# collabora/WhisperLive

Measured on AMD Instinct MI355X. Metric: real-time factor (xRT), Whisper-small 30 s window (p50 chunk latency in p50_chunk_latency_ms), higher is better.
Workload: dtype f16 (MFMA operands; f32 accumulate, f32 residual stream, f32 log-mel); 1 GPU; configs[1]: Whisper-small.en, 1 stream per GPU, one 30 s window per stream per step (480000 samples 16 kHz f32 resident in HBM -> log-mel -> encoder -> beam-5 decode, 64 generated tokens forced by suppressing EOT), seeded random weights; streams_per_gpu=1, beam_size=5, decode_steps=64

## Files before the change

### whisperlive_amd/_lib.py

```python
from __future__ import annotations

import ctypes as C
import os
import shutil
import subprocess
from pathlib import Path

import numpy as np

PKG_DIR = Path(__file__).resolve().parent
CSRC = PKG_DIR / "csrc"
DEFAULT_LIB = PKG_DIR / "libwlx.so"
LIB_PATH = Path(os.environ["WLX_LIB"]).resolve() if os.environ.get("WLX_LIB") else DEFAULT_LIB
SOURCES = ["pack.hip", "logmel.hip", "gemm.hip", "attention.hip", "decoder.hip", "align.hip", "dec_gemv.hip", "dec_vocab.hip", "search.hip", "host.hip", "engine.hip", "engine_decode.hip", "engine_debug.hip", "resample.hip", "flac.hip", "vad.hip", "mt.hip", "mt_engine.hip", "spk.hip", "spk_engine.hip",
           "kernel_hooks.hip"]
EXPORTS = [
    "wlx_abi_version", "wlx_last_error", "wlx_engine_create", "wlx_engine_destroy", "wlx_engine_spec",
    "wlx_slot_create", "wlx_slot_destroy", "wlx_logmel", "wlx_pcm_put", "wlx_pcm_put_frames", "wlx_pcm_put_frames_split", "wlx_flac_probe", "wlx_pcm_put_flac", "wlx_pcm_put_flac_split", "wlx_pcm_get", "wlx_logmel_resident", "wlx_features_get", "wlx_features_set", "wlx_encode",
    "wlx_encoder_output_get", "wlx_generate", "wlx_generate_ex", "wlx_detect_language", "wlx_align", "wlx_align_batch", "wlx_timings_get", "wlx_sync",
    "wlx_vad_create", "wlx_vad_destroy", "wlx_vad_probs",
    "wlx_ring_create", "wlx_ring_destroy", "wlx_ring_append", "wlx_ring_state", "wlx_vad_probs_resident", "wlx_vad_segments", "wlx_logmel_ring",
    "wlx_logmel_chunks", "wlx_logmel_chunks_multi", "wlx_vad_probs_pcm", "wlx_vad_probs_batch", "wlx_vad_probs_pcm_batch",
    "wlx_mt_create", "wlx_mt_destroy", "wlx_mt_slot_create", "wlx_mt_slot_destroy", "wlx_mt_translate",
    "wlx_spk_create", "wlx_spk_destroy", "wlx_spk_embed", "wlx_spk_embed_batch", "wlx_spk_embed_pcm_batch", "wlx_spk_embed_ring_batch",
    "wlx_debug_logits_get", "wlx_debug_decode_logits", "wlx_debug_search", "wlx_debug_search_batch", "wlx_debug_time_decode_step", "wlx_debug_profile_step", "wlx_debug_trace_step",
    "wlx_mt_debug_encode", "wlx_mt_debug_decode_logits", "wlx_mt_debug_timings", "wlx_mt_debug_attn", "wlx_mt_debug_topk",
    "wlx_mt_debug_embed",
    "wlx_spk_debug_timings", "wlx_spk_debug_fbank", "wlx_spk_debug_conv", "wlx_spk_debug_pool",
    "wlx_spk_debug_conv_batch", "wlx_spk_debug_pool_batch",
    "wlx_debug_layernorm", "wlx_debug_attn_encoder", "wlx_debug_dec_cross_attn", "wlx_debug_dec_self_attn", "wlx_debug_gemm",
    "wlx_debug_dec_gemv", "wlx_debug_dec_cq_cross_attn",
    "wlx_debug_resample", "wlx_debug_resample_split", "wlx_debug_resample_timed", "wlx_debug_flac_decode", "wlx_debug_flac_timings",
    "wlx_debug_dtw", "wlx_debug_align_post", "wlx_debug_align_timings",
]


HIPCC_EXTRA = ["-mllvm", "-amdgpu-mfma-vgpr-form=1"]


class WlxError(RuntimeError):
    code = None


class wlx_spec(C.Structure):
    _fields_ = [(n, C.c_int32) for n in
                ("n_mels", "d_model", "n_heads", "enc_layers", "dec_layers", "ffn", "vocab", "n_audio_ctx", "n_text_ctx")]


class wlx_tensor(C.Structure):
    _fields_ = [("name", C.c_char_p), ("data", C.c_void_p), ("ndim", C.c_int32), ("shape", C.c_int64 * 4),
                ("on_device", C.c_int32)]


class wlx_token_ids(C.Structure):
    _fields_ = [(n, C.c_int32) for n in ("sot", "eot", "no_timestamps", "timestamp_begin", "no_speech", "blank")]


class wlx_gen_opts(C.Structure):
    _fields_ = [
        ("beam_size", C.c_int32), ("patience", C.c_float), ("num_hypotheses", C.c_int32),
        ("length_penalty", C.c_float), ("repetition_penalty", C.c_float), ("no_repeat_ngram_size", C.c_int32),
        ("max_length", C.c_int32), ("suppress_blank", C.c_int32), ("suppress_tokens", C.POINTER(C.c_int32)),
        ("n_suppress_tokens", C.c_int32), ("max_initial_timestamp_index", C.c_int32), ("sampling_topk", C.c_int32),
        ("sampling_temperature", C.c_float), ("seed", C.c_uint64), ("ids", wlx_token_ids),
    ]


class wlx_timings(C.Structure):
    _fields_ = [("logmel_ms", C.c_float), ("encode_ms", C.c_float), ("generate_ms", C.c_float), ("decode_steps", C.c_int32)]

# ... 32 lines not shown
ALIGN_MAX_MEDIAN = 15
ERR_ARG = 1
ERR_STATE = 4
LM_MAXRANGES = 256
PCM_F32, PCM_S16 = 0, 1
PCM_MAX_CHANNELS = 8
RESAMPLE_MAX_RATIO = 640
RESAMPLE_MIN_TILE = 64
RESAMPLE_MAX_LDS = 64 * 1024


class wlx_debug_gemm_args(C.Structure):
    _fields_ = ([(n, C.c_int32) for n in ("zbatch", "M", "N", "K", "KT", "conv3_cin", "mode", "force_form", "d", "rows_per_item")] +
                [("qscale", C.c_float), ("reserved", C.c_int32)] +
                [(n, C.c_int64) for n in ("lda", "strideA", "a_len", "ldc", "strideC", "c_len", "ldx", "strideX", "x_len",
                                          "ldk", "kv_item_stride_k", "kv_layer_stride_k", "k_len",
                                          "ldvt", "kv_item_stride_v", "kv_layer_stride_v", "v_len")])


class wlx_debug_dec_gemv_args(C.Structure):
    _fields_ = ([(n, C.c_int32) for n in ("in_mode", "out_mode", "xsrc", "M", "K", "KT", "N", "busy_device", "KTS", "H", "R", "d")] +
                [("qscale", C.c_float), ("reserved", C.c_int32)] +
                [(n, C.c_int64) for n in ("ldx", "ldxh", "ldyh", "ldy", "ldxres", "cache_row_stride", "slab_stride",
                                          "x_len", "xh_len", "part_o_len", "part_ml_len", "slab_len", "tok_emb_len", "pos_emb_len",
                                          "yh_len", "y_len", "xres_len", "kc_len", "vc_len", "intok_len")])


class wlx_mt_gen_opts(C.Structure):
    _fields_ = [("num_beams", C.c_int32), ("max_length", C.c_int32), ("early_stopping", C.c_int32),
                ("length_penalty", C.c_float), ("no_repeat_ngram_size", C.c_int32), ("forced_eos_token_id", C.c_int32)]


_extra_ok = None


def _hipcc() -> str:
    hipcc = shutil.which("hipcc") or "/opt/rocm/bin/hipcc"
    if not os.path.exists(hipcc):
        raise WlxError("hipcc not found: cannot build libwlx.so (ROCm toolchain required)")
    return hipcc


def _compile(out: Path, defines=(), verbose: bool = False, force: bool = False) -> Path:
    global _extra_ok
    from concurrent.futures import ThreadPoolExecutor
    hipcc = _hipcc()
    defines = list(defines)
    hdrs = list(CSRC.glob("*.h")) + [PKG_DIR.parent / "include" / "wlx.h"]
    hdr_time = max(h.stat().st_mtime for h in hdrs)
    base = [hipcc, "--offload-arch=gfx950", "-O3", "-std=c++17", "-fPIC"] + [f"-D{d}" for d in defines]

    def objects(extra):
        tag = "_".join(["base" if extra else "agpr"] + [d.replace("=", "-") for d in defines])
        odir = CSRC / ".obj" / tag
        odir.mkdir(parents=True, exist_ok=True)

        def one(src):
            obj = odir / (src + ".o")
            sp = CSRC / src
            if not force and obj.exists() and obj.stat().st_mtime >= max(sp.stat().st_mtime, hdr_time):
                return obj, None
            tmp = obj.with_name(obj.name + f".tmp{os.getpid()}")
            proc = subprocess.run(base + extra + ["-c", str(sp), "-o", str(tmp)], capture_output=True, text=True)
            if verbose and (proc.stdout or proc.stderr):
                print(proc.stdout, proc.stderr)
            if proc.returncode != 0:
                if tmp.exists():
                    tmp.unlink()
                return None, proc
            os.replace(tmp, obj)
            return obj, None
        with ThreadPoolExecutor(max_workers=min(len(SOURCES), os.cpu_count() or 4)) as ex:
            return list(ex.map(one, SOURCES))

    for extra in ([HIPCC_EXTRA, []] if _extra_ok is not False else [[]]):
        res = objects(extra)
        bad = [p for o, p in res if o is None]
        if not bad:
            if extra:
                _extra_ok = True
            tmp = out.with_name(out.name + f".tmp{os.getpid()}")
            proc = subprocess.run([hipcc, "--offload-arch=gfx950", "-shared", "-fPIC", "-o", str(tmp)] + [str(o) for o, _ in res],
                                  capture_output=True, text=True)
            if proc.returncode != 0:
                if tmp.exists():
                    tmp.unlink()
                raise WlxError(f"hipcc link failed ({proc.returncode}):\n{proc.stderr[-4000:]}")
            os.replace(tmp, out)
            return out
        err = bad[0].stderr
        if extra and ("Unknown command line argument" in err or "unknown argument" in err.lower()):
            _extra_ok = False
            print(f"[wlx build] this hipcc rejects {' '.join(HIPCC_EXTRA)}: building with MFMA accumulators in AGPR form")
            continue
        raise WlxError(f"hipcc failed ({bad[0].returncode}):\n{err[-4000:]}")
    raise WlxError("hipcc failed")


def _fresh(out: Path) -> bool:
    deps = [CSRC / s for s in SOURCES] + list(CSRC.glob("*.h")) + [PKG_DIR.parent / "include" / "wlx.h"]
    return out.exists() and all(out.stat().st_mtime >= d.stat().st_mtime for d in deps)


def build_trace() -> Path:
    out = PKG_DIR / "libwlx_trace.so"
    return out if _fresh(out) else _compile(out, ["WLX_TRACE"])


def build_ab() -> Path:
    out = PKG_DIR / "libwlx_ab.so"
    return out if _fresh(out) else _compile(out, ["WLX_AB"])


def build_variant(name: str, defines) -> Path:
    out = PKG_DIR / name
    return out if _fresh(out) else _compile(out, list(defines))


def build(force: bool = False, verbose: bool = False) -> Path:
    if not force and _fresh(DEFAULT_LIB):
        return DEFAULT_LIB
    return _compile(DEFAULT_LIB, (), verbose, force=force)


_lib = None


def load() -> C.CDLL:
    global _lib
    if _lib is not None:
        return _lib
    if not LIB_PATH.exists():
        raise WlxError(f"{LIB_PATH} not built: run `python -c 'import __graft_entry__ as g; g.build()'` "
                       "(hipcc --offload-arch=gfx950). whisperlive_amd has no CPU fallback.")
    try:
        lib = C.CDLL(str(LIB_PATH))
    except OSError as e:
        raise WlxError(f"cannot load {LIB_PATH}: {e}") from e
    missing = [s for s in EXPORTS if not hasattr(lib, s)]
    if missing:
        raise WlxError(f"libwlx.so lacks symbols {missing}")
    i32, i64, f32p, i32p, vp = C.c_int32, C.c_int64, C.POINTER(C.c_float), C.POINTER(C.c_int32), C.c_void_p
    lib.wlx_abi_version.restype = i32
    lib.wlx_last_error.restype = C.c_char_p
    lib.wlx_engine_create.argtypes = [C.POINTER(wlx_spec), C.POINTER(wlx_tensor), i32, i32, C.POINTER(vp)]
    lib.wlx_engine_destroy.argtypes = [vp]
    lib.wlx_engine_destroy.restype = None
    lib.wlx_engine_spec.argtypes = [vp, C.POINTER(wlx_spec)]
    lib.wlx_slot_create.argtypes = [vp, i32, i32, i32p]
# ... 131 lines not shown
```

### whisperlive_amd/csrc/dec_gemv.hip

```cpp
#include "dec_gemv_internal.h"
#include <algorithm>
#include <cstdio>

namespace wlx {

#define GV_CH 6

template <int MT, int NTB, int IN>
__global__ __launch_bounds__(512) void dec_gemv_kernel(GemvParams p) {
    if (p.done && *p.done) return;
    extern __shared__ __attribute__((aligned(16))) float smem[];
    const int tid = threadIdx.x, wave = tid >> 6, lane = tid & 63, c = lane & 15, g = lane >> 4;
    const int nw = blockDim.x >> 6;
    const int KT = p.KT;
    const int KTW = (KT + nw - 1) / nw;
    const int kt0 = wave * KTW;
    const int kt1 = (kt0 + KTW < KT) ? kt0 + KTW : KT;
    const int NT_total = (p.N + 15) >> 4;

    const half_t* wbase[NTB];
#pragma unroll
    for (int i = 0; i < NTB; ++i) {
        int nt = blockIdx.x * NTB + i;
        if (nt >= NT_total) nt = NT_total - 1;
// ... 290 lines not shown
template <int P, class F>
__device__ __forceinline__ void stage_rows_f16_wave(const half_t* __restrict__ X, long ldx, int M, int K, half_t* xs, int ldxs, int lane,
                                                    F&& after_first_loads) {
    const int kv8 = K >> 3, total = M * kv8;
    {
        int m_[P], k_[P];
        f16x8 v_[P];
#pragma unroll
        for (int q = 0; q < P; ++q) {
            int u = lane + 64 * q;
            if (u >= total) u = (q == 0) ? total - 1 : (lane + 64 * (q - 1) < total ? lane + 64 * (q - 1) : total - 1);
            m_[q] = u / kv8; k_[q] = u - m_[q] * kv8;
            v_[q] = ld_f16x8(X + (long)m_[q] * ldx + k_[q] * 8);
        }
        after_first_loads();
#pragma unroll
        for (int q = 0; q < P; ++q) *reinterpret_cast<f16x8*>(xs + m_[q] * ldxs + k_[q] * 8) = v_[q];
    }
#pragma unroll 1
    for (int u0 = lane + 64 * P; u0 < total; u0 += 128) {
        const int u1 = u0 + 64;
        const int m0 = u0 / kv8, k0 = u0 - m0 * kv8;
        const int uc = (u1 < total) ? u1 : u0;
        const int m1 = uc / kv8, k1 = uc - m1 * kv8;
        const f16x8 v0 = ld_f16x8(X + (long)m0 * ldx + k0 * 8);
        const f16x8 v1 = ld_f16x8(X + (long)m1 * ldx + k1 * 8);
        *reinterpret_cast<f16x8*>(xs + m0 * ldxs + k0 * 8) = v0;
        *reinterpret_cast<f16x8*>(xs + m1 * ldxs + k1 * 8) = v1;
    }
}


template <int CH, int LNV, int IN, int OUT, int NTB, int MT, int XS>
__global__ __launch_bounds__((IN == GEMV_IN_LN || OUT == GEMV_OUT_SLAB || MT > 1 || CH > 6 || IN == GEMV_IN_XATTN) ? 512 : 1024) void dec_gemv2_kernel(GemvParams p_in) {
    GemvParams p = p_in;
    int tile = blockIdx.x;
    if (p_in.Mtot > 0) {
        int zc = (int)blockIdx.z;
        if (p_in.rt_nz > 0) {
            const int lin = (int)blockIdx.x, t = lin >> 3;
            const int tq = (int)(((unsigned)t * (unsigned)p_in.rt_magic) >> 16);
            zc = t - tq * p_in.rt_nz;
            tile = tq * 8 + (lin & 7);
            if (tile >= p_in.rt_tiles) return;
        }
        const int CHK = p_in.chunk;
        const int r0 = zc * CHK;
        p.M = (p_in.Mtot - r0 < CHK) ? p_in.Mtot - r0 : CHK;
        if (p.emb_token) p.emb_token += r0;
        if (p.X) p.X += (long)r0 * p.ldx;
        if (p.Xh) p.Xh += (long)r0 * p.ldxh;
        if (p.Yh) p.Yh += (long)r0 * p.ldyh;
        if (p.Y) p.Y += (long)r0 * p.ldy;
        if (p.Xres) p.Xres += (long)r0 * p.ldxres;
        if (p.slab) p.slab += (long)r0 * ((IN == GEMV_IN_LN) ? p.ldx : p.ldxres);
        if (p.row_cache) p.row_cache += r0;
        if (p.row_pos) p.row_pos += r0;
    }
    static_assert(XS == GEMV_X_PLAIN || IN == GEMV_IN_LN || (IN == GEMV_IN_F16 && OUT == GEMV_OUT_RESID && NTB == 1),
                  "slab / embedding sources: LayerNorm prologue or residual epilogue only");
    static_assert(OUT != GEMV_OUT_SLAB || (IN == GEMV_IN_F16 && NTB == 1), "K-split form: fp16 rows in");
    extern __shared__ __attribute__((aligned(16))) float smem[];
    const int tid = threadIdx.x, lane = tid & 63, c = lane & 15, g = lane >> 4;
    const int wave = __builtin_amdgcn_readfirstlane(tid >> 6);
    const int nw = p.nwm;
    WLX_TR_BEGIN();
    constexpr int NP = NTB * MT;
    constexpr bool LNT = (LNV == 15);
    constexpr int NV = LNT ? 2 : LNV;
    const bool tail_on = !LNT || lane < 32;
    const int tback = LNT ? (tail_on ? 0 : lane) : 0;
    (void)tail_on; (void)tback;
    float* accred = smem;
    half_t* xs = reinterpret_cast<half_t*>(smem + nw * NP * 256);

    const bool streams = (IN != GEMV_IN_XATTN) || wave < nw;
    const int kx0 = (streams ? wave : 0) * p.KTW;
    const int ks0 = (OUT == GEMV_OUT_SLAB) ? (int)blockIdx.y * p.KTS : 0;
    const int kw0 = ks0 + kx0;
    const half_t* wp = p.Wp + ((long)(tile * NTB) * p.KT + kw0) * 512 + lane * 8;
    const long wstep = (long)p.KT * 512;
    f16x8 wf[CH][NTB];
    auto load_weights = [&]() {
        asm volatile("" ::: "memory");
        const half_t* wq = streams ? wp : p.Wp + ((long)(tile * NTB) * p.KT + ks0) * 512 + lane * 8;
        const long js = streams ? 512 : 0, is = streams ? wstep : 0;
#pragma unroll
        for (int j = 0; j < CH; ++j)
#pragma unroll
            for (int i = 0; i < NTB; ++i) wf[j][i] = ld_nt_f16x8(wq + i * is + j * js);
    };

    int crow[MT];
#pragma unroll
    for (int mt = 0; mt < MT; ++mt) crow[mt] = (mt * 16 + c < p.M) ? mt * 16 + c : p.M - 1;
    const int pair0 = (wave < NP) ? wave : 0;
    const int nt_e = tile * NTB + pair0 / MT;
    const int n_e = nt_e * 16 + g * 4;
    int row_e = (pair0 % MT) * 16 + c;
    if (row_e >= p.M) row_e = p.M - 1;
    float4 bias_e = make_float4(0.f, 0.f, 0.f, 0.f), res_e = bias_e;
    int rc_e = 0, rp_e = 0;
    if constexpr (OUT != GEMV_OUT_F32) bias_e = *reinterpret_cast<const float4*>(p.bias + n_e);
    if constexpr (OUT == GEMV_OUT_RESID) res_e = *reinterpret_cast<const float4*>(p.Xres + (long)row_e * p.ldxres + n_e);
    if constexpr (OUT == GEMV_OUT_QKV) { rc_e = p.row_cache[row_e]; rp_e = p.row_pos[row_e]; }
    float4 slab_e[(OUT == GEMV_OUT_RESID && XS == GEMV_X_SLABS) ? WLX_FC2_KS : 1];
    if constexpr (OUT == GEMV_OUT_RESID && XS == GEMV_X_SLABS) {
#pragma unroll
        for (int sl = 0; sl < WLX_FC2_KS; ++sl)
            slab_e[sl] = *reinterpret_cast<const float4*>(p.slab + sl * p.slab_stride + (long)row_e * p.ldxres + n_e);
    }
    if constexpr (OUT == GEMV_OUT_SLAB) { if (blockIdx.y != 0) bias_e = make_float4(0.f, 0.f, 0.f, 0.f); }

    f32x4 acc[NTB][MT];
#pragma unroll
    for (int i = 0; i < NTB; ++i)
#pragma unroll
        for (int mt = 0; mt < MT; ++mt) acc[i][mt] = (f32x4){0.f, 0.f, 0.f, 0.f};
    f16x8 xf[CH][MT];

    if constexpr (IN == GEMV_IN_F16) {
        const half_t* xr[MT];
        int xstep;
        if (MT == 1 && p.xstage) {
            const int Ks = (OUT == GEMV_OUT_SLAB) ? p.KTS * 32 : p.K;
            const int ldxs = Ks + 8;
            stage_rows_f16_wave<(CH * 4 * 5 + 63) / 64>(p.Xh + (ks0 + kx0) * 32, p.ldxh, p.M, p.KTW * 32, xs + kx0 * 32, ldxs, lane, [&]() { load_weights(); });
            WLX_TR_MARK(1);
            __builtin_amdgcn_fence(__ATOMIC_RELEASE, "wavefront");
            __builtin_amdgcn_wave_barrier();
            __builtin_amdgcn_fence(__ATOMIC_ACQUIRE, "wavefront");
            xr[0] = xs + crow[0] * ldxs + kx0 * 32 + g * 8;
            xstep = 32;
        } else {
#pragma unroll
            for (int mt = 0; mt < MT; ++mt) xr[mt] = p.Xh + (long)crow[mt] * p.ldxh + kw0 * 32 + g * 8;
            xstep = 32;
        }
#pragma unroll
        for (int j = 0; j < CH; ++j)
#pragma unroll
            for (int mt = 0; mt < MT; ++mt) xf[j][mt] = *reinterpret_cast<const f16x8*>(xr[mt] + j * xstep);
        if (!(MT == 1 && p.xstage)) load_weights();
#pragma unroll 1
        for (int ch = 1; ch < p.NCH; ++ch) {
// ... 401 lines not shown
            }
            *reinterpret_cast<float4*>(p.Xres + (long)c * p.ldxres + n_e) =
                make_float4(res_e.x + o0, res_e.y + o1, res_e.z + o2, res_e.w + o3);
        } else if constexpr (OUT == GEMV_OUT_SLAB) {
            *reinterpret_cast<float4*>(p.slab + blockIdx.y * p.slab_stride + (long)c * p.ldxres + n_e) = make_float4(o0, o1, o2, o3);
        } else {
            if (n_e < p.d) {
                const f16x4 h = {(half_t)(o0 * p.qscale), (half_t)(o1 * p.qscale), (half_t)(o2 * p.qscale), (half_t)(o3 * p.qscale)};
                *reinterpret_cast<f16x4*>(p.Yh + (long)c * p.ldyh + n_e) = h;
            } else {
                const f16x4 h = {(half_t)o0, (half_t)o1, (half_t)o2, (half_t)o3};
                const bool isk = n_e < 2 * p.d;
                half_t* dst = (isk ? p.Kc : p.Vc) + (long)rc_e * p.cache_row_stride + (long)rp_e * p.d + (n_e - (isk ? p.d : 2 * p.d));
                *reinterpret_cast<f16x4*>(dst) = h;
            }
        }
    }
    }
    WLX_TR_MARK(5);
    WLX_TR_END_WAVES(p.trc);
}

std::atomic<bool> g_lds_optin_refused{false};
void lds_optin(const void* kernel, std::atomic<signed char> (&granted)[64], const char* what) {
    int dev = 0;
    (void)hipGetDevice(&dev);
    if (dev < 0 || dev >= 64 || granted[dev].load(std::memory_order_acquire) != 0) return;
    const hipError_t e = hipFuncSetAttribute(kernel, hipFuncAttributeMaxDynamicSharedMemorySize, WLX_G2_LDS_MAX);
    if (e == hipSuccess) { granted[dev].store(1, std::memory_order_release); return; }
    (void)hipGetLastError();
    g_lds_optin_refused.store(true);
    fprintf(stderr, "[wlx] device %d refused %d KiB of dynamic LDS (%s): %s to the general kernel\n", dev, WLX_G2_LDS_MAX / 1024, hipGetErrorString(e), what);
}
template <int CH, int LNV, int IN, int OUT, int NTB, int MT, int XS>
static void g2_launch(dim3 grid, dim3 block, size_t shm, hipStream_t s, const GemvParams& p) {
    if (shm > 64 * 1024) {
        static std::atomic<signed char> granted[64] = {};
        lds_optin(reinterpret_cast<const void*>(&dec_gemv2_kernel<CH, LNV, IN, OUT, NTB, MT, XS>), granted, "batched decode projections fall back");
    }
    hipLaunchKernelGGL((dec_gemv2_kernel<CH, LNV, IN, OUT, NTB, MT, XS>), grid, block, shm, s, p);
}
void dispatch_bug(const char* kernel, hipStream_t s) {
    fprintf(stderr, "[wlx] launch_dec_gemv: no %s instantiation for a configuration its probe accepted\n", kernel);
    (void)hipLaunchKernel(nullptr, dim3(1), dim3(64), nullptr, 0, s);
}

struct Gemv2Cfg { bool ok, xstage; int nw, CH, NCH, LNV, NTB, MT; size_t shm; };
static bool gemv2_cfg_waves(const GemvParams& p, int KTf, Gemv2Cfg& c) {
    const int cap = (p.in_mode == GEMV_IN_F16 && p.out_mode != GEMV_OUT_SLAB && p.M <= 16) ? 16 : 8;
    int best_nch = 1 << 30;
    const bool ln_wide = p.in_mode == GEMV_IN_LN && p.M <= 8 && p.Mtot == 0 && (p.K == 1024 || p.K == 1280);
    if (p.in_mode == GEMV_IN_LN && p.xsrc != GEMV_X_PLAIN && !(ln_wide && p.out_mode == GEMV_OUT_QKV)) {
        const int want = std::min(p.M, 8);
        for (int CH = 6; CH >= 2; --CH) {
            if (KTf % CH || KTf / CH > 8 || KTf / CH < want) continue;
            best_nch = 1; c.nw = KTf / CH; c.CH = CH; c.NCH = 1;
            break;
        }
    } else {
        const int chmax = (p.in_mode == GEMV_IN_F16 && p.M <= 16 && p.Mtot == 0) ? 12 : ln_wide ? 10 : 6;
        for (int CH = chmax; CH >= 4; --CH) {
            if (CH != 12 && CH != 10 && CH != 8 && CH > 6) continue;
            if (ln_wide && CH > 6 && CH * 128 != p.K) continue;
            if (KTf % CH) continue;
            const int q = KTf / CH;
            for (int nw = std::min(CH > 6 ? std::min(cap, 8) : cap, q); nw >= 1; --nw) {
                if (q % nw) continue;
                if (CH > 6 && nw > 4 && (nw & 3)) break;
                const int nch = q / nw;
                if (nch < best_nch) { best_nch = nch; c.nw = nw; c.CH = CH; c.NCH = nch; }
                break;
            }
        }
// ... 17 lines not shown
    int NTB = (p.out_mode == GEMV_OUT_F32 && p.N > 8192) ? 2 : 1;
    if (p.in_mode == GEMV_IN_LN && p.out_mode == GEMV_OUT_GELU_F16 && p.xsrc == GEMV_X_PLAIN && (p.N + 15) / 16 > 256 && ((p.N + 15) / 16) % 2 == 0) NTB = 2;
    if (p.Mtot > 0 && p.rt_nz > 0 && p.in_mode == GEMV_IN_LN && p.xsrc == GEMV_X_PLAIN &&
        (p.out_mode == GEMV_OUT_GELU_F16 || p.out_mode == GEMV_OUT_QKV) && (p.N + 15) / 16 >= 128 && ((p.N + 15) / 16) % 2 == 0) NTB = 2;
    if (NTB == 2 && p.Mtot > 0 && p.rt_nz > 0 && ((p.N + 15) / 16) % 4 == 0 && p.M <= 16) NTB = 4;
    if (p.busy_device && p.Mtot > 0 && p.rt_nz > 0 && p.M <= 16 && p.in_mode == GEMV_IN_F16 && p.out_mode == GEMV_OUT_RESID && p.xsrc == GEMV_X_PLAIN && ((p.N + 15) / 16) % 2 == 0) NTB = 2;
    return NTB;
}
static bool gemv2_cfg_staging(const GemvParams& p, int KTf, Gemv2Cfg& c) {
    c.MT = (p.M + 15) / 16;
    c.shm = sizeof(float) * (size_t)c.nw * c.NTB * c.MT * 256;
    const size_t xs_bytes = (size_t)p.M * (KTf * 32 + 8) * sizeof(half_t);
    if (c.NTB == 2 && p.out_mode == GEMV_OUT_GELU_F16 && c.shm + xs_bytes > WLX_G2_LDS_MAX) {
        c.NTB = 1;
        c.shm = sizeof(float) * (size_t)c.nw * c.NTB * c.MT * 256;
    }
    c.xstage = true;
    const size_t xstage_max = (p.Mtot > 0 && p.rt_nz > 0) ? (size_t)WLX_G2_LDS_MAX : (size_t)64 * 1024;
    if (p.in_mode == GEMV_IN_F16 && (c.MT > 1 || c.shm + xs_bytes > xstage_max)) c.xstage = false;
    if (c.xstage) c.shm += xs_bytes;
    if (c.shm > WLX_G2_LDS_MAX) return false;
    if (c.shm > 64 * 1024 && g_lds_optin_refused.load(std::memory_order_relaxed)) return false;
    return true;
}
static Gemv2Cfg gemv2_cfg(const GemvParams& p) {
    Gemv2Cfg c{};
    if (g_decode_v1 || p.M > 48 || p.M < 1) return c;
    if (p.bias ? (p.N & 15) != 0 : p.out_mode != GEMV_OUT_F32) return c;
    const bool combo = (p.in_mode == GEMV_IN_LN && (p.out_mode == GEMV_OUT_QKV || p.out_mode == GEMV_OUT_F16 ||
                                                    p.out_mode == GEMV_OUT_GELU_F16 || p.out_mode == GEMV_OUT_F32)) ||
                       (p.in_mode != GEMV_IN_LN && p.out_mode == GEMV_OUT_RESID) ||
                       (p.in_mode == GEMV_IN_F16 && p.out_mode == GEMV_OUT_SLAB);
    if (!combo || p.K != p.KT * 32) return c;
    if (p.xsrc != GEMV_X_PLAIN) {
        const bool ln_ok = p.in_mode == GEMV_IN_LN && p.out_mode == GEMV_OUT_QKV;
        const bool res_ok = p.in_mode == GEMV_IN_F16 && p.out_mode == GEMV_OUT_RESID && p.xsrc == GEMV_X_SLABS;
        if (!(ln_ok || res_ok)) return c;
    }
    int KTf = p.KT;
    if (p.out_mode == GEMV_OUT_SLAB) {
        if (p.KTS < 1 || p.KT % p.KTS || p.KT / p.KTS != WLX_FC2_KS) return c;
        KTf = p.KTS;
    }
    if (!gemv2_cfg_waves(p, KTf, c)) return c;
    c.NTB = gemv2_cfg_tiles(p);
    c.ok = gemv2_cfg_staging(p, KTf, c);
    return c;
}

template <int CH_, int LNV_, int IN_, int OUT_, int NTB_, int MT_, int XS_>
struct G2Args { static constexpr int CH = CH_, LNV = LNV_, IN = IN_, OUT = OUT_, NTB = NTB_, MT = MT_, XS = XS_; };
enum G2Rows { G2_LN_XS, G2_LN_PLAIN, G2_NO_LN };
template <int CH, int LNV, int OUT, int MT, int NTBMAX, class Leaf>
static bool gemv2_dispatch_ntb(const Gemv2Cfg& c, Leaf& leaf) {
    if (c.NTB == 1) return leaf(G2Args<CH, LNV, GEMV_IN_LN, OUT, 1, MT, GEMV_X_PLAIN>{});
    if constexpr (NTBMAX >= 2) { if (c.NTB == 2) return leaf(G2Args<CH, LNV, GEMV_IN_LN, OUT, 2, MT, GEMV_X_PLAIN>{}); }
    if constexpr (NTBMAX >= 4 && MT == 1) { if (c.NTB == 4) return leaf(G2Args<CH, LNV, GEMV_IN_LN, OUT, 4, 1, GEMV_X_PLAIN>{}); }
    return false;
}
template <int ROWS, int CH, int LNV, int MT, class Leaf>
static bool gemv2_dispatch_modes(const GemvParams& p, const Gemv2Cfg& c, Leaf& leaf) {
    if constexpr (ROWS == G2_LN_XS) {
        if (p.out_mode != GEMV_OUT_QKV || c.NTB != 1) return false;
        if (p.xsrc == GEMV_X_SLABS) return leaf(G2Args<CH, LNV, GEMV_IN_LN, GEMV_OUT_QKV, 1, MT, GEMV_X_SLABS>{});
        return p.xsrc == GEMV_X_EMBED && leaf(G2Args<CH, LNV, GEMV_IN_LN, GEMV_OUT_QKV, 1, MT, GEMV_X_EMBED>{});
    } else if constexpr (ROWS == G2_LN_PLAIN) {
// ... 15 lines not shown
        if (p.xsrc == GEMV_X_SLABS) return c.NTB == 1 && leaf(G2Args<CH, 1, GEMV_IN_F16, GEMV_OUT_RESID, 1, MT, GEMV_X_SLABS>{});
        if (p.xsrc != GEMV_X_PLAIN) return false;
        if (c.NTB == 1) return leaf(G2Args<CH, 1, GEMV_IN_F16, GEMV_OUT_RESID, 1, MT, GEMV_X_PLAIN>{});
        if constexpr (MT == 1) { if (c.NTB == 2) return leaf(G2Args<CH, 1, GEMV_IN_F16, GEMV_OUT_RESID, 2, 1, GEMV_X_PLAIN>{}); }
        return false;
    }
}
template <int ROWS, int CH, int LNV, int MTMAX, class Leaf>
static bool gemv2_dispatch_pair(const GemvParams& p, const Gemv2Cfg& c, Leaf& leaf) {
    if (c.CH != CH || c.LNV != LNV) return false;
    if (c.MT == 1) return gemv2_dispatch_modes<ROWS, CH, LNV, 1>(p, c, leaf);
    if constexpr (MTMAX == 3) return c.MT == 2 ? gemv2_dispatch_modes<ROWS, CH, LNV, 2>(p, c, leaf) : c.MT == 3 && gemv2_dispatch_modes<ROWS, CH, LNV, 3>(p, c, leaf);
    return false;
}
template <class Leaf>
static bool gemv2_dispatch(const GemvParams& p, const Gemv2Cfg& c, Leaf leaf) {
    if (p.in_mode == GEMV_IN_LN && p.xsrc != GEMV_X_PLAIN)
        return gemv2_dispatch_pair<G2_LN_XS, 4, 3, 3>(p, c, leaf) || gemv2_dispatch_pair<G2_LN_XS, 3, 3, 3>(p, c, leaf) || gemv2_dispatch_pair<G2_LN_XS, 2, 2, 3>(p, c, leaf) ||
               gemv2_dispatch_pair<G2_LN_XS, 4, 4, 3>(p, c, leaf) || gemv2_dispatch_pair<G2_LN_XS, 5, 5, 3>(p, c, leaf) || gemv2_dispatch_pair<G2_LN_XS, 2, 15, 1>(p, c, leaf) ||
               gemv2_dispatch_pair<G2_LN_XS, 6, 3, 1>(p, c, leaf) || gemv2_dispatch_pair<G2_LN_XS, 8, 4, 1>(p, c, leaf) || gemv2_dispatch_pair<G2_LN_XS, 10, 5, 1>(p, c, leaf);
    if (p.in_mode == GEMV_IN_LN)
        return gemv2_dispatch_pair<G2_LN_PLAIN, 6, 3, 3>(p, c, leaf) || gemv2_dispatch_pair<G2_LN_PLAIN, 5, 5, 3>(p, c, leaf) || gemv2_dispatch_pair<G2_LN_PLAIN, 4, 2, 3>(p, c, leaf) ||
               gemv2_dispatch_pair<G2_LN_PLAIN, 4, 4, 3>(p, c, leaf) || gemv2_dispatch_pair<G2_LN_PLAIN, 10, 5, 1>(p, c, leaf) || gemv2_dispatch_pair<G2_LN_PLAIN, 8, 4, 1>(p, c, leaf) ||
               gemv2_dispatch_pair<G2_LN_PLAIN, 2, 15, 1>(p, c, leaf);
    return gemv2_dispatch_pair<G2_NO_LN, 12, 1, 1>(p, c, leaf) || gemv2_dispatch_pair<G2_NO_LN, 10, 1, 1>(p, c, leaf) || gemv2_dispatch_pair<G2_NO_LN, 8, 1, 1>(p, c, leaf) ||
           gemv2_dispatch_pair<G2_NO_LN, 6, 1, 3>(p, c, leaf) || gemv2_dispatch_pair<G2_NO_LN, 5, 1, 3>(p, c, leaf) || gemv2_dispatch_pair<G2_NO_LN, 4, 1, 3>(p, c, leaf);
}
static bool gemv2_ok(const GemvParams& p, Gemv2Cfg* out) {
    const Gemv2Cfg c = gemv2_cfg(p);
    if (!c.ok || !gemv2_dispatch(p, c, [](auto) { return true; })) return false;
    if (out) *out = c;
    return true;
}
static void gemv2_launch(const GemvParams& p0, const Gemv2Cfg& c, hipStream_t s) {
    GemvParams p = p0;
    p.KTW = c.CH * c.NCH; p.NCH = c.NCH; p.xstage = c.xstage ? 1 : 0; p.nwm = c.nw;
#ifdef WLX_TRACE
    { static thread_local char nm[512][48]; const int q = g_trace_seq < 512 ? g_trace_seq : 511;
      snprintf(nm[q], 48, "gemv2<%d,%d,%d> N%d K%d", p.in_mode, p.out_mode, p.xsrc, p.N, p.K); p.trc = trace_next(nm[q]); }
#endif
    const int NT_total = (p.N + 15) / 16;
    if (p.Mtot > 0 && p.chunk <= 0) p.chunk = 48;
    dim3 grid((NT_total + c.NTB - 1) / c.NTB, p.out_mode == GEMV_OUT_SLAB ? p.KT / p.KTS : 1, p.Mtot > 0 ? (p.Mtot + p.chunk - 1) / p.chunk : 1), block(c.nw * 64);
    if (p.Mtot > 0 && p.rt_nz > 0) {
        p.rt_tiles = (int)grid.x;
        p.rt_magic = 65536 / p.rt_nz + 1;
        grid.x = ((grid.x + 7) / 8) * 8 * p.rt_nz;
        grid.z = 1;
    }
    if (p.in_mode == GEMV_IN_XATTN && c.MT > 1) {
        const int want = (p.M * p.H * 8 + 63) / 64;
        block.x = 64 * std::max(c.nw, std::min(8, want));
    }
    const bool launched = gemv2_dispatch(p, c, [&](auto a) { using A = decltype(a); g2_launch<A::CH, A::LNV, A::IN, A::OUT, A::NTB, A::MT, A::XS>(grid, block, c.shm, s, p); return true; });
    if (!launched) dispatch_bug("dec_gemv2_kernel", s);
}
static GemvParams gemv_chunked(const GemvParams& p) {
    constexpr int rt_max = WLX_MAX_DEC_ROWS;
    int rt_chunk = 16;
    if (p.in_mode == GEMV_IN_F16 && p.out_mode == GEMV_OUT_RESID && p.xsrc == GEMV_X_PLAIN && !p.busy_device && p.M > 64) {
        static const int n_cu = [] { int dev = 0, n = 256; (void)hipGetDevice(&dev); hipDeviceProp_t pr; if (hipGetDeviceProperties(&pr, dev) == hipSuccess && pr.multiProcessorCount > 0) n = pr.multiProcessorCount; return n; }();
        const int tiles = (p.N + 15) / 16;
        double best = 1e300;
        for (int mt = 1; mt <= 3; ++mt) {
            const long wgs = (long)tiles * ((p.M + 16 * mt - 1) / (16 * mt));
            const double cost = (double)((wgs + n_cu - 1) / n_cu) * (1.0 + 0.35 * (mt - 1));
            if (cost < best - 1e-9) { best = cost; rt_chunk = 16 * mt; }
        }
    }
    GemvParams q = p;
    if (p.Mtot != 0 || p.in_mode == GEMV_IN_XATTN) return q;
    const bool ln_wide4 = rt_chunk == 16 && p.M > 32 && p.in_mode == GEMV_IN_LN && p.xsrc == GEMV_X_PLAIN && (p.out_mode == GEMV_OUT_QKV || p.out_mode == GEMV_OUT_GELU_F16) &&
                          (p.N & 15) == 0 && ((p.N >> 4) & 3) == 0;
    const bool rt_shape = p.N <= 1536 || (long)p.N * p.K <= 3200000L || ln_wide4;
    if (!g_decode_v1 && p.M > rt_chunk && p.M <= rt_max && rt_shape) { q.Mtot = p.M; q.M = rt_chunk; q.chunk = rt_chunk; q.rt_nz = (p.M + rt_chunk - 1) / rt_chunk; }
    else if (p.M > 48 && p.xsrc != GEMV_X_EMBED) { q.Mtot = p.M; q.M = 48; q.chunk = 48; }
    return q;
}

int dec_gemv_slab_split(int M, int K, int N) {
    if (WLX_FC2_KS < 2) return 0;
    if (g_decode_v1 || M < 1 || K % 32 || (K / 32) % WLX_FC2_KS || K < 2048) return 0;
    GemvParams p0{};
    p0.in_mode = GEMV_IN_F16; p0.out_mode = GEMV_OUT_SLAB; p0.M = M; p0.K = K; p0.KT = K / 32; p0.N = N; p0.KTS = p0.KT / WLX_FC2_KS;
    static const float dummy_bias = 0.f;
    p0.bias = &dummy_bias;
    const GemvParams p = gemv_chunked(p0);
    Gemv2Cfg c;
    if (!gemv2_ok(p, &c) || (p.M <= 16 && !c.xstage)) return 0;
    return WLX_FC2_KS;
}

template <int MT, int NTB>
static void gemv_dispatch_in(const GemvParams& p, dim3 grid, dim3 block, size_t shm, hipStream_t s) {
    switch (p.in_mode) {
        case GEMV_IN_LN: hipLaunchKernelGGL((dec_gemv_kernel<MT, NTB, GEMV_IN_LN>), grid, block, shm, s, p); break;
        case GEMV_IN_F16: hipLaunchKernelGGL((dec_gemv_kernel<MT, NTB, GEMV_IN_F16>), grid, block, shm, s, p); break;
        default: hipLaunchKernelGGL((dec_gemv_kernel<MT, NTB, GEMV_IN_XATTN>), grid, block, shm, s, p); break;
    }
}

bool dec_gemv_is_lean(const GemvParams& p) { return vocab2_ok(p) || gemv2_ok(gemv_chunked(p), nullptr); }

const char* dec_gemv_kernel_name(const GemvParams& p_any) {
    if (vocab2_ok(p_any)) return vocab2_kernel_name(p_any);
    static thread_local char buf[64];
    const GemvParams p = gemv_chunked(p_any);
    Gemv2Cfg c2;
    if (gemv2_ok(p, &c2)) {
        gemv2_dispatch(p, c2, [&](auto a) { using A = decltype(a); snprintf(buf, sizeof(buf), "dec_gemv2_kernel<%d, %d, %d, %d, %d, %d, %d>", A::CH, A::LNV, A::IN, A::OUT, A::NTB, A::MT, A::XS); return true; });
        return buf;
    }
    const int MT = (p.M + 15) / 16;
    snprintf(buf, sizeof(buf), "dec_gemv_kernel<%d, %d, %d>", MT > 4 ? 4 : MT, MT == 1 ? 2 : 1, p.in_mode);
    return buf;
}

void launch_dec_gemv(const GemvParams& p, hipStream_t s) {
    if (vocab2_ok(p)) { vocab2_launch(p, s); return; }
    Gemv2Cfg c2;
    const GemvParams pc = gemv_chunked(p);
    if (gemv2_ok(pc, &c2)) { gemv2_launch(pc, c2, s); return; }
    if (p.M > 16 * WLX_MAX_MT) {
        const int CHK = (p.in_mode == GEMV_IN_XATTN && p.R > 0) ? (16 * WLX_MAX_MT / p.R) * p.R : 16 * WLX_MAX_MT;
        for (int r0 = 0; r0 < p.M; r0 += CHK) {
            GemvParams q = p;
            q.M = std::min(CHK, p.M - r0);
            if (q.X) q.X += (long)r0 * q.ldx;
            if (q.Xh) q.Xh += (long)r0 * q.ldxh;
            if (q.Yh) q.Yh += (long)r0 * q.ldyh;
            if (q.Y) q.Y += (long)r0 * q.ldy;
            if (q.Xres) q.Xres += (long)r0 * q.ldxres;
            if (q.row_cache) q.row_cache += r0;
            if (q.row_pos) q.row_pos += r0;
// ... 27 lines not shown
```

### whisperlive_amd/csrc/dec_gemv_internal.h

```cpp
#pragma once
#include "decoder.h"
#include <atomic>

namespace wlx {

#define WLX_G2_LDS_MAX (152 * 1024)
extern std::atomic<bool> g_lds_optin_refused;
void lds_optin(const void* kernel, std::atomic<signed char> (&granted)[64], const char* what);
void dispatch_bug(const char* kernel, hipStream_t s);

bool vocab2_ok(const GemvParams& p);
void vocab2_launch(const GemvParams& p, hipStream_t s);
const char* vocab2_kernel_name(const GemvParams& p);

}
```

Before: 1158 xRT (audio s / wall s).

## Preload decode GEMV argument head into SGPRs via kernarg preload

```diff
diff --git a/whisperlive_amd/_lib.py b/whisperlive_amd/_lib.py
--- a/whisperlive_amd/_lib.py
+++ b/whisperlive_amd/_lib.py
@@ -36,6 +36,8 @@
 
 
 HIPCC_EXTRA = ["-mllvm", "-amdgpu-mfma-vgpr-form=1"]
+KERNARG_PRELOAD = ["-mllvm", "-amdgpu-kernarg-preload-count=14"]
+KERNARG_PRELOAD_SOURCES = ("dec_gemv.hip", "decoder.hip", "search.hip")
 
 
 class WlxError(RuntimeError):
@@ -134,6 +136,7 @@
 
 
 _extra_ok = None
+_preload_ok = None
 
 
 def _hipcc() -> str:
@@ -144,7 +147,7 @@
 
 
 def _compile(out: Path, defines=(), verbose: bool = False, force: bool = False) -> Path:
-    global _extra_ok
+    global _extra_ok, _preload_ok
     from concurrent.futures import ThreadPoolExecutor
     hipcc = _hipcc()
     defines = list(defines)
@@ -152,18 +155,21 @@
     hdr_time = max(h.stat().st_mtime for h in hdrs)
     base = [hipcc, "--offload-arch=gfx950", "-O3", "-std=c++17", "-fPIC"] + [f"-D{d}" for d in defines]
 
-    def objects(extra):
-        tag = "_".join(["base" if extra else "agpr"] + [d.replace("=", "-") for d in defines])
+    want_pre = "WLX_KERNARG_HEAD=0" not in defines
+
+    def objects(extra, preload):
+        tag = "_".join(["base" if extra else "agpr"] + (["nopre"] if want_pre and not preload else []) + [d.replace("=", "-") for d in defines])
         odir = CSRC / ".obj" / tag
         odir.mkdir(parents=True, exist_ok=True)
 
         def one(src):
-            obj = odir / (src + ".o")
+            pre = KERNARG_PRELOAD if (preload and src in KERNARG_PRELOAD_SOURCES) else []
+            obj = odir / (src + (".pre.o" if pre else ".o"))
             sp = CSRC / src
             if not force and obj.exists() and obj.stat().st_mtime >= max(sp.stat().st_mtime, hdr_time):
                 return obj, None
             tmp = obj.with_name(obj.name + f".tmp{os.getpid()}")
-            proc = subprocess.run(base + extra + ["-c", str(sp), "-o", str(tmp)], capture_output=True, text=True)
+            proc = subprocess.run(base + extra + pre + ["-c", str(sp), "-o", str(tmp)], capture_output=True, text=True)
             if verbose and (proc.stdout or proc.stderr):
                 print(proc.stdout, proc.stderr)
             if proc.returncode != 0:
@@ -175,12 +181,16 @@
         with ThreadPoolExecutor(max_workers=min(len(SOURCES), os.cpu_count() or 4)) as ex:
             return list(ex.map(one, SOURCES))
 
-    for extra in ([HIPCC_EXTRA, []] if _extra_ok is not False else [[]]):
-        res = objects(extra)
+    for _attempt in range(3):
+        extra = HIPCC_EXTRA if _extra_ok is not False else []
+        preload = want_pre and _preload_ok is not False
+        res = objects(extra, preload)
         bad = [p for o, p in res if o is None]
         if not bad:
             if extra:
                 _extra_ok = True
+            if preload:
+                _preload_ok = True
             tmp = out.with_name(out.name + f".tmp{os.getpid()}")
             proc = subprocess.run([hipcc, "--offload-arch=gfx950", "-shared", "-fPIC", "-o", str(tmp)] + [str(o) for o, _ in res],
                                   capture_output=True, text=True)
@@ -191,9 +201,15 @@
             os.replace(tmp, out)
             return out
         err = bad[0].stderr
-        if extra and ("Unknown command line argument" in err or "unknown argument" in err.lower()):
-            _extra_ok = False
-            print(f"[wlx build] this hipcc rejects {' '.join(HIPCC_EXTRA)}: building with MFMA accumulators in AGPR form")
+        if (extra or preload) and ("Unknown command line argument" in err or "unknown argument" in err.lower()):
+            no_pre = preload and (KERNARG_PRELOAD[1].split("=")[0] in err or HIPCC_EXTRA[1].split("=")[0] not in err)
+            no_extra = bool(extra) and (HIPCC_EXTRA[1].split("=")[0] in err or KERNARG_PRELOAD[1].split("=")[0] not in err)
+            if no_pre:
+                _preload_ok = False
+                print(f"[wlx build] this hipcc rejects {' '.join(KERNARG_PRELOAD)}: the decode projections fetch their argument head themselves")
+            if no_extra:
+                _extra_ok = False
+                print(f"[wlx build] this hipcc rejects {' '.join(HIPCC_EXTRA)}: building with MFMA accumulators in AGPR form")
             continue
         raise WlxError(f"hipcc failed ({bad[0].returncode}):\n{err[-4000:]}")
     raise WlxError("hipcc failed")
@@ -217,6 +233,10 @@
 def build_variant(name: str, defines) -> Path:
     out = PKG_DIR / name
     return out if _fresh(out) else _compile(out, list(defines))
+
+
+def build_nohead() -> Path:
+    return build_variant("libwlx_nohead.so", ["WLX_KERNARG_HEAD=0"])
 
 
 def build(force: bool = False, verbose: bool = False) -> Path:
diff --git a/whisperlive_amd/csrc/dec_gemv.hip b/whisperlive_amd/csrc/dec_gemv.hip
--- a/whisperlive_amd/csrc/dec_gemv.hip
+++ b/whisperlive_amd/csrc/dec_gemv.hip
@@ -346,21 +346,65 @@
 
 
 template <int CH, int LNV, int IN, int OUT, int NTB, int MT, int XS>
-__global__ __launch_bounds__((IN == GEMV_IN_LN || OUT == GEMV_OUT_SLAB || MT > 1 || CH > 6 || IN == GEMV_IN_XATTN) ? 512 : 1024) void dec_gemv2_kernel(GemvParams p_in) {
+__global__ __launch_bounds__((IN == GEMV_IN_LN || OUT == GEMV_OUT_SLAB || MT > 1 || CH > 6 || IN == GEMV_IN_XATTN) ? 512 : 1024) void dec_gemv2_kernel(WLX_G2_HEAD_PARAMS GemvParams p_in) {
     GemvParams p = p_in;
+#if WLX_KERNARG_HEAD
+    p.Wp = h_wp; p.gamma = h_gamma; p.beta = h_beta;
+    p.M = h_dims & 0xff; p.nwm = (h_dims >> 8) & 0xff; p.KTW = (h_dims >> 16) & 0xff; p.xstage = (h_dims >> 24) & 1;
+    p.KT = h_kt & 0xff; p.KTS = (h_kt >> 8) & 0xff; p.K = p.KT * 32;
+    const int h_mtot = (int)((unsigned)h_kt >> 16);
+    if constexpr (IN == GEMV_IN_LN) {
+        if constexpr (XS != GEMV_X_EMBED) { p.X = static_cast<const float*>(h_rows); p.ldx = h_ld; }
+        if constexpr (XS == GEMV_X_SLABS) { p.slab = const_cast<float*>(static_cast<const float*>(h_aux)); p.slab_stride = h_aux_i; }
+    } else if constexpr (IN == GEMV_IN_F16) {
+        p.Xh = static_cast<const half_t*>(h_rows); p.ldxh = h_ld;
+    } else {
+        p.part_o = static_cast<const half_t*>(h_rows); p.part_ml = static_cast<const float*>(h_aux); p.R = h_aux_i & 0xffff; p.H = h_aux_i >> 16;
+    }
+#else
+    const int h_mtot = p_in.Mtot;
+#endif
     int tile = blockIdx.x;
-    if (p_in.Mtot > 0) {
+#if WLX_KERNARG_HEAD
+    int row0 = 0;
+#endif
+    if (h_mtot > 0) {
+#if WLX_KERNARG_HEAD
+        const __attribute__((address_space(4))) char* ka = (const __attribute__((address_space(4))) char*)__builtin_amdgcn_kernarg_segment_ptr();
+        asm volatile("" : "+s"(ka));
+        const __attribute__((address_space(4))) GemvParams& pc = *reinterpret_cast<const __attribute__((address_space(4))) GemvParams*>(ka + sizeof(GemvHead));
+#else
+        const GemvParams& pc = p_in;
+#endif
+        const int c_nz = pc.rt_nz, c_magic = pc.rt_magic, c_tiles = pc.rt_tiles, c_chunk = pc.chunk, c_mtot = pc.Mtot;
         int zc = (int)blockIdx.z;
-        if (p_in.rt_nz > 0) {
+        if (c_nz > 0) {
             const int lin = (int)blockIdx.x, t = lin >> 3;
-            const int tq = (int)(((unsigned)t * (unsigned)p_in.rt_magic) >> 16);
-            zc = t - tq * p_in.rt_nz;
+            const int tq = (int)(((unsigned)t * (unsigned)c_magic) >> 16);
+            zc = t - tq * c_nz;
             tile = tq * 8 + (lin & 7);
-            if (tile >= p_in.rt_tiles) return;
-        }
-        const int CHK = p_in.chunk;
+            if (tile >= c_tiles) return;
+        }
+        const int CHK = c_chunk;
         const int r0 = zc * CHK;
-        p.M = (p_in.Mtot - r0 < CHK) ? p_in.Mtot - r0 : CHK;
+        p.M = (c_mtot - r0 < CHK) ? c_mtot - r0 : CHK;
+#if WLX_KERNARG_HEAD
+        row0 = r0;
+    }
+    {
+        const long r0 = row0;
+        p.X += r0 * p.ldx; p.Xh += r0 * p.ldxh;
+        if constexpr (IN == GEMV_IN_LN) p.slab += r0 * p.ldx;
+        if constexpr (XS == GEMV_X_EMBED) { p.emb_token += r0; p.row_cache += r0; p.row_pos += r0; }
+    }
+    auto rebase_late = [&]() {
+        long r0 = row0;
+        asm volatile("" : "+s"(r0));
+        p.Yh += r0 * p.ldyh; p.Y += r0 * p.ldy; p.Xres += r0 * p.ldxres;
+        if constexpr (IN != GEMV_IN_LN) p.slab += r0 * p.ldxres;
+        if constexpr (XS != GEMV_X_EMBED) { p.row_cache += r0; p.row_pos += r0; }
+    };
+#else
         if (p.emb_token) p.emb_token += r0;
         if (p.X) p.X += (long)r0 * p.ldx;
         if (p.Xh) p.Xh += (long)r0 * p.ldxh;
@@ -371,6 +415,7 @@
         if (p.row_cache) p.row_cache += r0;
         if (p.row_pos) p.row_pos += r0;
     }
+#endif
     static_assert(XS == GEMV_X_PLAIN || IN == GEMV_IN_LN || (IN == GEMV_IN_F16 && OUT == GEMV_OUT_RESID && NTB == 1),
                   "slab / embedding sources: LayerNorm prologue or residual epilogue only");
     static_assert(OUT != GEMV_OUT_SLAB || (IN == GEMV_IN_F16 && NTB == 1), "K-split form: fp16 rows in");
@@ -395,16 +440,6 @@
     const half_t* wp = p.Wp + ((long)(tile * NTB) * p.KT + kw0) * 512 + lane * 8;
     const long wstep = (long)p.KT * 512;
     f16x8 wf[CH][NTB];
-    auto load_weights = [&]() {
-        asm volatile("" ::: "memory");
-        const half_t* wq = streams ? wp : p.Wp + ((long)(tile * NTB) * p.KT + ks0) * 512 + lane * 8;
-        const long js = streams ? 512 : 0, is = streams ? wstep : 0;
-#pragma unroll
-        for (int j = 0; j < CH; ++j)
-#pragma unroll
-            for (int i = 0; i < NTB; ++i) wf[j][i] = ld_nt_f16x8(wq + i * is + j * js);
-    };
-
     int crow[MT];
 #pragma unroll
     for (int mt = 0; mt < MT; ++mt) crow[mt] = (mt * 16 + c < p.M) ? mt * 16 + c : p.M - 1;
@@ -415,16 +450,40 @@
     if (row_e >= p.M) row_e = p.M - 1;
     float4 bias_e = make_float4(0.f, 0.f, 0.f, 0.f), res_e = bias_e;
     int rc_e = 0, rp_e = 0;
-    if constexpr (OUT != GEMV_OUT_F32) bias_e = *reinterpret_cast<const float4*>(p.bias + n_e);
-    if constexpr (OUT == GEMV_OUT_RESID) res_e = *reinterpret_cast<const float4*>(p.Xres + (long)row_e * p.ldxres + n_e);
-    if constexpr (OUT == GEMV_OUT_QKV) { rc_e = p.row_cache[row_e]; rp_e = p.row_pos[row_e]; }
     float4 slab_e[(OUT == GEMV_OUT_RESID && XS == GEMV_X_SLABS) ? WLX_FC2_KS : 1];
-    if constexpr (OUT == GEMV_OUT_RESID && XS == GEMV_X_SLABS) {
-#pragma unroll
-        for (int sl = 0; sl < WLX_FC2_KS; ++sl)
-            slab_e[sl] = *reinterpret_cast<const float4*>(p.slab + sl * p.slab_stride + (long)row_e * p.ldxres + n_e);
-    }
-    if constexpr (OUT == GEMV_OUT_SLAB) { if (blockIdx.y != 0) bias_e = make_float4(0.f, 0.f, 0.f, 0.f); }
+    auto load_epilogue_operands = [&]() {
+        int row_q = row_e;
+#if WLX_KERNARG_HEAD
+        rebase_late();
+        asm volatile("" : "+v"(row_q));
+#endif
+        if constexpr (OUT != GEMV_OUT_F32) bias_e = *reinterpret_cast<const float4*>(p.bias + n_e);
+        if constexpr (OUT == GEMV_OUT_RESID) res_e = *reinterpret_cast<const float4*>(p.Xres + (long)row_q * p.ldxres + n_e);
+        if constexpr (OUT == GEMV_OUT_QKV) { rc_e = p.row_cache[row_q]; rp_e = p.row_pos[row_q]; }
+        if constexpr (OUT == GEMV_OUT_RESID && XS == GEMV_X_SLABS) {
+#pragma unroll
+            for (int sl = 0; sl < WLX_FC2_KS; ++sl)
+                slab_e[sl] = *reinterpret_cast<const float4*>(p.slab + sl * p.slab_stride + (long)row_q * p.ldxres + n_e);
+        }
+        if constexpr (OUT == GEMV_OUT_SLAB) { if (blockIdx.y != 0) bias_e = make_float4(0.f, 0.f, 0.f, 0.f); }
+    };
+#if !WLX_KERNARG_HEAD
+    load_epilogue_operands();
+#endif
+    auto load_weights = [&]() {
+        asm volatile("" ::: "memory");
+        const half_t* wq = streams ? wp : p.Wp + ((long)(tile * NTB) * p.KT + ks0) * 512 + lane * 8;
+        const long js = streams ? 512 : 0, is = streams ? wstep : 0;
+#pragma unroll
+        for (int j = 0; j < CH; ++j)
+#pragma unroll
+            for (int i = 0; i < NTB; ++i) wf[j][i] = ld_nt_f16x8(wq + i * is + j * js);
+#if WLX_KERNARG_HEAD
+        asm volatile("" ::: "memory");
+        __builtin_amdgcn_sched_barrier(0);
+        load_epilogue_operands();
+#endif
+    };
 
     f32x4 acc[NTB][MT];
 #pragma unroll
@@ -892,13 +951,39 @@
     g_lds_optin_refused.store(true);
     fprintf(stderr, "[wlx] device %d refused %d KiB of dynamic LDS (%s): %s to the general kernel\n", dev, WLX_G2_LDS_MAX / 1024, hipGetErrorString(e), what);
 }
+static bool g2_head_fits(const GemvParams& p) {
+    const long lim = 0x7fffffffL;
+    return p.KT >= 0 && p.KT <= 255 && p.KTS >= 0 && p.KTS <= 255 && p.Mtot >= 0 && p.Mtot <= 65535 && p.M >= 0 && p.M <= 255 &&
+           p.ldx >= 0 && p.ldx <= lim && p.ldxh >= 0 && p.ldxh <= lim && p.slab_stride >= 0 && p.slab_stride <= lim &&
+           (p.in_mode != GEMV_IN_XATTN || (p.R >= 0 && p.R <= 0xffff && p.H >= 0 && p.H <= 0x7fff));
+}
+bool g2_head(const GemvParams& p, GemvHead* h) {
+    if (!g2_head_fits(p) || p.nwm < 0 || p.nwm > 255 || p.KTW < 0 || p.KTW > 255) return false;
+    *h = GemvHead{};
+    h->gamma = p.gamma; h->beta = p.beta; h->wp = p.Wp;
+    h->dims = p.M | (p.nwm << 8) | (p.KTW << 16) | ((p.xstage ? 1 : 0) << 24);
+    h->kt = p.KT | (p.KTS << 8) | (int)((unsigned)p.Mtot << 16);
+    if (p.in_mode == GEMV_IN_LN) {
+        if (p.xsrc != GEMV_X_EMBED) { h->rows = p.X; h->ld = (int)p.ldx; }
+        if (p.xsrc == GEMV_X_SLABS) { h->aux = p.slab; h->aux_i = (int)p.slab_stride; }
+    } else if (p.in_mode == GEMV_IN_F16) {
+        h->rows = p.Xh; h->ld = (int)p.ldxh;
+    } else {
+        h->rows = p.part_o; h->aux = p.part_ml; h->aux_i = p.R | (p.H << 16);
+    }
+    return true;
+}
 template <int CH, int LNV, int IN, int OUT, int NTB, int MT, int XS>
 static void g2_launch(dim3 grid, dim3 block, size_t shm, hipStream_t s, const GemvParams& p) {
+#if WLX_KERNARG_HEAD
+    GemvHead h;
+    if (!g2_head(p, &h)) { dispatch_bug("dec_gemv2_kernel (argument head)", s); return; }
+#endif
     if (shm > 64 * 1024) {
         static std::atomic<signed char> granted[64] = {};
         lds_optin(reinterpret_cast<const void*>(&dec_gemv2_kernel<CH, LNV, IN, OUT, NTB, MT, XS>), granted, "batched decode projections fall back");
     }
-    hipLaunchKernelGGL((dec_gemv2_kernel<CH, LNV, IN, OUT, NTB, MT, XS>), grid, block, shm, s, p);
+    hipLaunchKernelGGL((dec_gemv2_kernel<CH, LNV, IN, OUT, NTB, MT, XS>), grid, block, shm, s, WLX_G2_HEAD_ARGS(h) p);
 }
 void dispatch_bug(const char* kernel, hipStream_t s) {
     fprintf(stderr, "[wlx] launch_dec_gemv: no %s instantiation for a configuration its probe accepted\n", kernel);
@@ -982,6 +1067,9 @@
                        (p.in_mode != GEMV_IN_LN && p.out_mode == GEMV_OUT_RESID) ||
                        (p.in_mode == GEMV_IN_F16 && p.out_mode == GEMV_OUT_SLAB);
     if (!combo || p.K != p.KT * 32) return c;
+#if WLX_KERNARG_HEAD
+    if (!g2_head_fits(p)) return c;
+#endif
     if (p.xsrc != GEMV_X_PLAIN) {
         const bool ln_ok = p.in_mode == GEMV_IN_LN && p.out_mode == GEMV_OUT_QKV;
         const bool res_ok = p.in_mode == GEMV_IN_F16 && p.out_mode == GEMV_OUT_RESID && p.xsrc == GEMV_X_SLABS;
@@ -1063,15 +1151,18 @@
     if (out) *out = c;
     return true;
 }
+static void gemv2_launch_fields(GemvParams& p, const Gemv2Cfg& c) {
+    p.KTW = c.CH * c.NCH; p.NCH = c.NCH; p.xstage = c.xstage ? 1 : 0; p.nwm = c.nw;
+    if (p.Mtot > 0 && p.chunk <= 0) p.chunk = 48;
+}
 static void gemv2_launch(const GemvParams& p0, const Gemv2Cfg& c, hipStream_t s) {
     GemvParams p = p0;
-    p.KTW = c.CH * c.NCH; p.NCH = c.NCH; p.xstage = c.xstage ? 1 : 0; p.nwm = c.nw;
+    gemv2_launch_fields(p, c);
 #ifdef WLX_TRACE
     { static thread_local char nm[512][48]; const int q = g_trace_seq < 512 ? g_trace_seq : 511;
       snprintf(nm[q], 48, "gemv2<%d,%d,%d> N%d K%d", p.in_mode, p.out_mode, p.xsrc, p.N, p.K); p.trc = trace_next(nm[q]); }
 #endif
     const int NT_total = (p.N + 15) / 16;
-    if (p.Mtot > 0 && p.chunk <= 0) p.chunk = 48;
     dim3 grid((NT_total + c.NTB - 1) / c.NTB, p.out_mode == GEMV_OUT_SLAB ? p.KT / p.KTS : 1, p.Mtot > 0 ? (p.Mtot + p.chunk - 1) / p.chunk : 1), block(c.nw * 64);
     if (p.Mtot > 0 && p.rt_nz > 0) {
         p.rt_tiles = (int)grid.x;
@@ -1131,6 +1222,15 @@
     }
 }
 
+bool dec_gemv_head(const GemvParams& p_any, GemvHead* h, GemvParams* launched) {
+    if (vocab2_ok(p_any)) return false;
+    GemvParams p = gemv_chunked(p_any);
+    Gemv2Cfg c;
+    if (!gemv2_ok(p, &c)) return false;
+    gemv2_launch_fields(p, c);
+    *launched = p;
+    return g2_head(p, h);
+}
 bool dec_gemv_is_lean(const GemvParams& p) { return vocab2_ok(p) || gemv2_ok(gemv_chunked(p), nullptr); }
 
 const char* dec_gemv_kernel_name(const GemvParams& p_any) {
diff --git a/whisperlive_amd/csrc/dec_gemv_internal.h b/whisperlive_amd/csrc/dec_gemv_internal.h
--- a/whisperlive_amd/csrc/dec_gemv_internal.h
+++ b/whisperlive_amd/csrc/dec_gemv_internal.h
@@ -9,6 +9,21 @@
 void lds_optin(const void* kernel, std::atomic<signed char> (&granted)[64], const char* what);
 void dispatch_bug(const char* kernel, hipStream_t s);
 
+#ifndef WLX_KERNARG_HEAD
+#define WLX_KERNARG_HEAD 1
+#endif
+struct GemvHead { const void* rows; const void* aux; const float* gamma; const float* beta; const half_t* wp; int ld, aux_i, dims, kt; };
+static_assert(sizeof(GemvHead) == 56 && sizeof(GemvHead) % alignof(GemvParams) == 0, "14 dwords, the struct right behind them in the kernel-argument segment");
+#if WLX_KERNARG_HEAD
+#define WLX_G2_HEAD_PARAMS const void* h_rows, const void* h_aux, const float* h_gamma, const float* h_beta, const half_t* h_wp, int h_ld, int h_aux_i, int h_dims, int h_kt,
+#define WLX_G2_HEAD_ARGS(h) (h).rows, (h).aux, (h).gamma, (h).beta, (h).wp, (h).ld, (h).aux_i, (h).dims, (h).kt,
+#else
+#define WLX_G2_HEAD_PARAMS
+#define WLX_G2_HEAD_ARGS(h)
+#endif
+bool g2_head(const GemvParams& p, GemvHead* h);
+bool dec_gemv_head(const GemvParams& p_any, GemvHead* h, GemvParams* launched);
+
 bool vocab2_ok(const GemvParams& p);
 void vocab2_launch(const GemvParams& p, hipStream_t s);
 const char* vocab2_kernel_name(const GemvParams& p);
```

Measured after the change: 1202 xRT (audio s / wall s) (median of 6 runs). 3.8% higher.
